# MrGiovanni/R-Super

Hardware: AMD Instinct MI355X
Metric: CT voxels/sec/node (96³ patch, bs=2/GPU) (higher is better)
Workload: dtype bf16; 1 GPU; R-Super 3D UNet(base 32, 26 classes, BasicBlock/IN) full training step (fwd + masked BCE + Dice loss + bwd + clip + AdamW + EMA), 96^3 patches, batch 2/GPU (BASELINE.json configs[1]); global_batch=2, patch=96, parallelism=dp1, sanity_checks_form=device-side flags read one step late (train_ddp.StepGuard)

## Files before the change

include/rsuper_hip.h:

```cpp
#ifndef RSUPER_HIP_H
#define RSUPER_HIP_H
#include <stddef.h>
#include <stdint.h>
#ifdef __cplusplus
extern "C" {
#endif

#define RSUPER_F32 0
#define RSUPER_BF16 1
#define RSUPER_OK 0
#define RSUPER_ERR_ARG 1
#define RSUPER_ERR_LAUNCH 2
#define RSUPER_ERR_UNSUPPORTED 3
#define RSUPER_ERR_NO_DEVICE 4

const char* rsuper_version(void);
int rsuper_device_check(void);


size_t rsuper_conv3_packed_elems(int dtype, int ka, int kb, int n_cols, int bn);

int rsuper_conv3_pack_weights(int dtype, int mode, const float* wa, const float* wb, int ka, int kb, int na, int nb,
                              int bn, void* packed, void* stream);

// ... 177 lines not shown
int rsuper_mask_op(uint8_t* a, const uint8_t* b, long V, int op , void* stream);

int rsuper_unpack_bits(const uint8_t* packed, uint8_t* out, int B, int P, int C, long V, void* stream);
int rsuper_timer_event_create(void** ev);
int rsuper_timer_event_record(void* ev, void* stream);
int rsuper_timer_event_elapsed_ms(void* a, void* b, float* ms);
int rsuper_timer_event_destroy(void* ev);

int rsuper_unpack_bits_sel(const uint8_t* packed, uint8_t* out, int B, int P, int C, long V, const uint8_t* flags, const uint8_t* force, void* stream);
int rsuper_plane_any_bits(const uint8_t* packed, int B, int P, int C, long V, uint8_t* flags, void* stream);
int rsuper_zero_where(float* x, const uint8_t* m, long V, void* stream);
int rsuper_count(const uint8_t* m, long V, unsigned int* count, void* stream);

long rsuper_detection_workspace_bytes(int planes);
int rsuper_detection(const float* x, int planes, int Di, int Hi, int Wi, int Do, int Ho, int Wo, const double* thresholds, int nthr, int erode,
                     long long* volumes, double* max_prob, void* workspace, void* stream);
int rsuper_organ_mask_u8(const uint8_t* pred, int C, int D, int H, int W, int n, const int* lesion, const int* organ_a, const int* organ_b,
                         uint8_t* out, void* stream);
int rsuper_organ_mask_f32(const float* pred, int C, int D, int H, int W, int n, const int* lesion, const int* organ_a, const int* organ_b,
                          float* out, void* stream);
long rsuper_largest_component_workspace_bytes(int D, int H, int W);
int rsuper_largest_component(const void* mask, int is_u8, int D, int H, int W, uint8_t* out, void* workspace, void* stream);

int rsuper_surface_codes(const uint8_t* gt, const uint8_t* pred, int planes, int D, int H, int W, uint8_t* codes_gt, uint8_t* codes_pred,
                         int* bbox, long long* counts, void* stream);
long rsuper_edt3_workspace_bytes(int nz, int ny, int nx);
int rsuper_edt3(const uint8_t* codes, int Dc, int Hc, int Wc, int z0, int y0, int x0, int nz, int ny, int nx, double s0, double s1, double s2,
                double* out, void* workspace, long workspace_bytes, void* stream);
int rsuper_surfel_gather(const uint8_t* codes, int Dc, int Hc, int Wc, int z0, int y0, int x0, int nz, int ny, int nx, const double* sqdist,
                         const double* table, double* dist, double* area, long long* count, long capacity, void* stream);

#define RSUPER_AFFINE_MAX_VOLUMES 3
#define RSUPER_AFFINE_MAX_PLANES 64
int rsuper_affine_crop(const float* theta, const float* img, float* img_out, int B, int Ci, int D, int H, int W, int nvol,
                       const uint8_t* const* vols, uint8_t* const* vols_out, const int* planes, int d, int h, int w, const int* offsets,
                       void* stream);

#define RSUPER_BLUR_MAX_RADIUS 5
long rsuper_intensity_augment_workspace_bytes(int B, int D, int H, int W);
int rsuper_intensity_augment_launches(int B, const int* flags);
int rsuper_intensity_augment(const float* img, float* out, int B, int D, int H, int W, const int* flags, const float* scalars, const int* radius,
                             const float* taps, const unsigned long long* seeds, const float* noise, void* workspace, long workspace_bytes,
                             void* stream);

int rsuper_grad_sqnorm(int n, void* const* host_g, const size_t* host_numel, double* total_sq, void* stream);
int rsuper_clip_scale(int n, void* const* host_g, const size_t* host_numel, float max_norm, const double* total_sq, void* stream);
int rsuper_adamw_ema_step(int n, void* const* host_p, void* const* host_g, void* const* host_m, void* const* host_v,
                          void* const* host_ema, const size_t* host_numel, float lr, float beta1, float beta2, float eps,
                          float weight_decay, int step, float ema_alpha, float max_norm, const double* total_sq, void* stream);
int rsuper_adamw_ema_step_dyn(int n, void* const* host_p, void* const* host_g, void* const* host_m, void* const* host_v,
                              void* const* host_ema, const size_t* host_numel, float beta1, float beta2, float eps, float weight_decay,
                              float max_norm, const double* total_sq, const float* dyn, void* stream);

#ifdef __cplusplus
}
#endif
#endif
```

r-super_amd/csrc/api.hip:

```cpp
#include <string.h>
#include <math.h>
#include <stdlib.h>
#include "common.hpp"
#include "kernels.hpp"
#include "misc.hpp"
#include "loss.hpp"
#include "morph.hpp"
#include "optim.hpp"
#include "../../include/rsuper_hip.h"

#define ST(s) ((hipStream_t)(s))

static inline bool dt_ok(int dt) { return dt == RS_F32 || dt == RS_BF16; }
static inline bool ch_ok(int C, int ld) { return C >= 0 && (C % 8) == 0 && (ld % 8) == 0 && ld >= C; }
static inline bool bn_ok(int bn) { return bn == 32 || bn == 64 || bn == 96 || bn == 128; }
static inline int ntiles_for(int n_cols, int bn) { const int per = bn / 32; return ((n_cols + bn - 1) / bn) * per; }
static inline int pack_cols(int mode, int na, int nb) { return mode == 1 ? (nb ? (nb & 0xFFFF) : na) : na + nb; }
static inline bool pack_range_ok(int mode, int na, int nb) { return mode != 1 || nb == 0 || ((nb >> 16) % 32 == 0 && (nb & 0xFFFF) > 0 && (nb >> 16) + (nb & 0xFFFF) <= na); }

#include "igemm_plan.hpp"

template <typename F>
static int for_chunks(int n, void* const* p, void* const* g, void* const* m, void* const* v, void* const* e, const size_t* numel, F f) {
    for (int i0 = 0; i0 < n; i0 += RS_MT_MAX) {
// ... 713 lines not shown
int rsuper_plane_any(const uint8_t* m, long planes, long V, uint8_t* flags, void* stream) {
    if (!m || !flags || planes <= 0 || V <= 0 || ((uintptr_t)m & 15) || (V & 15 && planes > 1)) return RS_ERR_ARG;
    return rs_launch_plane_any(m, planes, V, flags, ST(stream));
}
int rsuper_mask_op(uint8_t* a, const uint8_t* b, long V, int op, void* stream) {
    if (!a || !b || op < 0 || op > 2) return RS_ERR_ARG;
    return rs_launch_mask_op(a, b, V, op, ST(stream));
}
int rsuper_zero_where(float* x, const uint8_t* m, long V, void* stream) {
    if (!x || !m) return RS_ERR_ARG;
    return rs_launch_zero_where(x, m, V, ST(stream));
}
int rsuper_count(const uint8_t* m, long V, unsigned int* count, void* stream) {
    if (!m || !count) return RS_ERR_ARG;
    return rs_launch_count(m, V, count, ST(stream));
}

int rsuper_grad_sqnorm(int n, void* const* host_g, const size_t* host_numel, double* total_sq, void* stream) {
    if (n <= 0 || !host_g || !host_numel || !total_sq) return RS_ERR_ARG;
    int first = 1;
    const int rc = for_chunks(n, nullptr, host_g, nullptr, nullptr, nullptr, host_numel, [&](const MTChunk& c) {
        const int r = rs_launch_sqnorm(c, total_sq, first, ST(stream));
        first = 0;
        return r;
    });
    if (rc == RS_OK && first) return rs_launch_zero_bytes(total_sq, sizeof(double), ST(stream));
    return rc;
}
int rsuper_clip_scale(int n, void* const* host_g, const size_t* host_numel, float max_norm, const double* total_sq, void* stream) {
    if (n <= 0 || !host_g || !host_numel || !total_sq) return RS_ERR_ARG;
    return for_chunks(n, nullptr, host_g, nullptr, nullptr, nullptr, host_numel, [&](const MTChunk& c) { return rs_launch_scale(c, max_norm, total_sq, ST(stream)); });
}
int rsuper_adamw_ema_step(int n, void* const* host_p, void* const* host_g, void* const* host_m, void* const* host_v,
                          void* const* host_ema, const size_t* host_numel, float lr, float beta1, float beta2, float eps,
                          float weight_decay, int step, float ema_alpha, float max_norm, const double* total_sq, void* stream) {
    if (n <= 0 || !host_p || !host_g || !host_m || !host_v || !host_numel || step < 1) return RS_ERR_ARG;
    AdamParams a;
    a.lr = lr; a.beta1 = beta1; a.beta2 = beta2; a.eps = eps; a.wd = weight_decay;
    a.step_size = (float)((double)lr / (1.0 - pow((double)beta1, (double)step)));
    a.sqrt_bc2 = (float)sqrt(1.0 - pow((double)beta2, (double)step));
    a.ema_alpha = ema_alpha; a.max_norm = max_norm; a.dyn = nullptr;
    return for_chunks(n, host_p, host_g, host_m, host_v, host_ema, host_numel, [&](const MTChunk& c) { return rs_launch_adamw_ema(c, a, total_sq, ST(stream)); });
}
int rsuper_adamw_ema_step_dyn(int n, void* const* host_p, void* const* host_g, void* const* host_m, void* const* host_v,
                              void* const* host_ema, const size_t* host_numel, float beta1, float beta2, float eps, float weight_decay,
                              float max_norm, const double* total_sq, const float* dyn, void* stream) {
    if (n <= 0 || !host_p || !host_g || !host_m || !host_v || !host_numel || !dyn) return RS_ERR_ARG;
    AdamParams a;
    a.lr = 0.f; a.beta1 = beta1; a.beta2 = beta2; a.eps = eps; a.wd = weight_decay;
    a.step_size = 0.f; a.sqrt_bc2 = 1.f; a.ema_alpha = 0.f; a.max_norm = max_norm; a.dyn = dyn;
    return for_chunks(n, host_p, host_g, host_m, host_v, host_ema, host_numel, [&](const MTChunk& c) { return rs_launch_adamw_ema(c, a, total_sq, ST(stream)); });
}

}
```

r-super_amd/csrc/optim.hip:

```cpp
#include "common.hpp"
#include "optim.hpp"

namespace {

__device__ __forceinline__ int find_tensor(const MTChunk& c, int blk, int& local) {
    int lo = 0, hi = c.n;
    while (hi - lo > 1) { const int mid = (lo + hi) >> 1; if (c.blk_start[mid] <= blk) lo = mid; else hi = mid; }
    local = blk - c.blk_start[lo];
    return lo;
}

constexpr int MT_ELEMS = 256 * 4 * 4;

__global__ __launch_bounds__(256) void sqnorm_kernel(MTChunk c, double* partial) {
    int local; const int ti = find_tensor(c, blockIdx.x, local);
    const float* g = (const float*)c.g[ti];
    const size_t n = c.numel[ti], base = (size_t)local * MT_ELEMS;
    float s = 0.f;
    if (base + MT_ELEMS <= n && (((uintptr_t)(g + base)) & 15) == 0) {
        const float4* g4 = (const float4*)(g + base);
#pragma unroll
        for (int k = 0; k < MT_ELEMS / 1024; ++k) { const float4 v = g4[threadIdx.x + 256 * k]; s += v.x * v.x + v.y * v.y + v.z * v.z + v.w * v.w; }
    } else {
#pragma unroll
        for (int k = 0; k < MT_ELEMS / 1024; ++k) {
            const size_t i = base + (size_t)(threadIdx.x + 256 * k) * 4;
            const float x = i < n ? g[i] : 0.f, y = i + 1 < n ? g[i + 1] : 0.f, z = i + 2 < n ? g[i + 2] : 0.f, w = i + 3 < n ? g[i + 3] : 0.f;
            s += x * x + y * y + z * z + w * w;
        }
    }
    s = wave_sum(s);
    __shared__ float red[4];
    if ((threadIdx.x & 63) == 0) red[threadIdx.x >> 6] = s;
    __syncthreads();
    if (threadIdx.x == 0) partial[blockIdx.x] = (double)red[0] + (double)red[1] + (double)red[2] + (double)red[3];
}

__global__ __launch_bounds__(256) void sqnorm_reduce_kernel(const double* partial, int n, double* total, int first) {
    __shared__ double red[256];
    double s = 0.0;
    for (int i = threadIdx.x; i < n; i += 256) s += partial[i];
    red[threadIdx.x] = s;
    __syncthreads();
    for (int o = 128; o > 0; o >>= 1) {
        if ((int)threadIdx.x < o) red[threadIdx.x] += red[threadIdx.x + o];
        __syncthreads();
    }
    if (threadIdx.x == 0) *total = first ? red[0] : *total + red[0];
}

__global__ __launch_bounds__(256) void adamw_ema_kernel(MTChunk c, AdamParams a, const double* total_sq) {
    int local; const int ti = find_tensor(c, blockIdx.x, local);
    float* p = (float*)c.p[ti]; const float* g = (const float*)c.g[ti];
    float* m = (float*)c.m[ti]; float* v = (float*)c.v[ti]; float* e = (float*)c.ema[ti];
    const size_t n = c.numel[ti], base = (size_t)local * MT_ELEMS;
    if (a.dyn) { a.lr = a.dyn[0]; a.step_size = a.dyn[1]; a.sqrt_bc2 = a.dyn[2]; a.ema_alpha = a.dyn[3]; }
    float coef = 1.f;
    if (total_sq) {
        const float norm = (float)sqrt(*total_sq);
        if (!(norm <= 3.0e38f)) return;
        coef = fminf(a.max_norm / (norm + 1e-6f), 1.f);
    }
    for (size_t i = base + threadIdx.x; i < base + MT_ELEMS && i < n; i += 256) {
        const float gi = g[i] * coef;
        float pi = p[i] * (1.f - a.lr * a.wd);
        const float mi = a.beta1 * m[i] + (1.f - a.beta1) * gi;
        const float vi = a.beta2 * v[i] + (1.f - a.beta2) * gi * gi;
        const float denom = sqrtf(vi) / a.sqrt_bc2 + a.eps;
        pi -= a.step_size * (mi / denom);
        p[i] = pi; m[i] = mi; v[i] = vi;
        if (e) e[i] = a.ema_alpha * e[i] + (1.f - a.ema_alpha) * pi;
    }
}

__global__ __launch_bounds__(256) void scale_kernel(MTChunk c, float max_norm, const double* total_sq) {
    int local; const int ti = find_tensor(c, blockIdx.x, local);
    float* g = (float*)c.g[ti];
    const size_t n = c.numel[ti], base = (size_t)local * MT_ELEMS;
    const float coef = fminf(max_norm / ((float)sqrt(*total_sq) + 1e-6f), 1.f);
    for (size_t i = base + threadIdx.x; i < base + MT_ELEMS && i < n; i += 256) g[i] *= coef;
}

__global__ __launch_bounds__(256) void zero_bytes_kernel(unsigned char* p, size_t bytes) {
    const size_t nv = bytes / 16, stride = (size_t)gridDim.x * 256;
    for (size_t i = (size_t)blockIdx.x * 256 + threadIdx.x; i < nv; i += stride) ((uint4*)p)[i] = make_uint4(0, 0, 0, 0);
    if (blockIdx.x == 0) for (size_t i = nv * 16 + threadIdx.x; i < bytes; i += 256) p[i] = 0;
}

}

int rs_launch_zero_bytes(void* p, size_t bytes, hipStream_t st) {
    if (!bytes) return RS_OK;
    const size_t nv = bytes / 16;
    size_t blocks = (nv + 255) / 256;
    if (blocks < 1) blocks = 1;
    if (blocks > 4096) blocks = 4096;
    const bool aligned = (((uintptr_t)p) & 15) == 0;
    if (!aligned) return RS_ERR_ARG;
    hipLaunchKernelGGL(zero_bytes_kernel, dim3((unsigned)blocks), dim3(256), 0, st, (unsigned char*)p, bytes);
    return rs_check_launch();
}
int rs_mt_blocks(size_t numel) { return (int)((numel + MT_ELEMS - 1) / MT_ELEMS); }

int rs_launch_sqnorm(const MTChunk& c, double* total, int first, hipStream_t st) {
    static double* ws[16] = {};
    constexpr int WS_BLOCKS = 1 << 16;
    int dev = 0;
    if (hipGetDevice(&dev) != hipSuccess || dev < 0 || dev >= 16) return RS_ERR_LAUNCH;
    if (!ws[dev] && hipMalloc((void**)&ws[dev], (size_t)WS_BLOCKS * sizeof(double)) != hipSuccess) return RS_ERR_LAUNCH;
    const int blocks = c.blk_start[c.n];
    if (blocks > WS_BLOCKS) return RS_ERR_UNSUPPORTED;
    hipLaunchKernelGGL(sqnorm_kernel, dim3(blocks), dim3(256), 0, st, c, ws[dev]);
    hipLaunchKernelGGL(sqnorm_reduce_kernel, dim3(1), dim3(256), 0, st, (const double*)ws[dev], blocks, total, first);
    return rs_check_launch();
}
int rs_launch_adamw_ema(const MTChunk& c, const AdamParams& a, const double* total_sq, hipStream_t st) {
    hipLaunchKernelGGL(adamw_ema_kernel, dim3(c.blk_start[c.n]), dim3(256), 0, st, c, a, total_sq);
    return rs_check_launch();
}
int rs_launch_scale(const MTChunk& c, float max_norm, const double* total_sq, hipStream_t st) {
    hipLaunchKernelGGL(scale_kernel, dim3(c.blk_start[c.n]), dim3(256), 0, st, c, max_norm, total_sq);
    return rs_check_launch();
}
```

r-super_amd/csrc/optim.hpp:

```cpp
#pragma once
#include <hip/hip_runtime.h>
#include <stddef.h>
#include <stdint.h>

#define RS_MT_MAX 36
struct MTChunk {
    int n;
    void* p[RS_MT_MAX]; void* g[RS_MT_MAX]; void* m[RS_MT_MAX]; void* v[RS_MT_MAX]; void* ema[RS_MT_MAX];
    size_t numel[RS_MT_MAX];
    int blk_start[RS_MT_MAX + 1];
};
struct AdamParams {
    float lr, beta1, beta2, eps, wd;
    float step_size;
    float sqrt_bc2;
    float ema_alpha;
    float max_norm;
    const float* dyn;
};
int rs_mt_blocks(size_t numel);
int rs_launch_sqnorm(const MTChunk& c, double* total, int first, hipStream_t st);
int rs_launch_zero_bytes(void* p, size_t bytes, hipStream_t st);
int rs_launch_adamw_ema(const MTChunk& c, const AdamParams& a, const double* total_sq, hipStream_t st);
int rs_launch_scale(const MTChunk& c, float max_norm, const double* total_sq, hipStream_t st);
```

r-super_amd/hip/lib.py:

```python
import ctypes
import os
from ctypes import c_int, c_long, c_longlong, c_size_t, c_float, c_double, c_void_p, c_uint32, c_uint

_HERE = os.path.dirname(os.path.abspath(__file__))
SO_PATH = os.path.join(os.path.dirname(_HERE), 'csrc', 'librsuper_hip.so')

F32, BF16 = 0, 1
BLUR_MAX_RADIUS = 5
_LIB = None

P = c_void_p
_SIGS = {
    'rsuper_version': (ctypes.c_char_p, []),
    'rsuper_device_check': (c_int, []),
    'rsuper_conv3_packed_elems': (c_size_t, [c_int] * 5),
    'rsuper_conv3_pack_weights': (c_int, [c_int, c_int, P, P, c_int, c_int, c_int, c_int, c_int, P, P]),
    'rsuper_conv3_pack_weights_batch': (c_int, [c_int, c_int, P, P, P, P, P, P]),
    'rsuper_conv3_tiles': (c_int, [c_int] * 3),
    'rsuper_conv3_variant': (c_int, [c_int]),
    'rsuper_conv3_wgrad2_min_tiles': (c_int, [c_int]),
    'rsuper_conv3_plan': (c_int, [c_int] * 11 + [P]),
    'rsuper_conv3_box_bn': (c_int, [c_int] * 6),
    'rsuper_conv3_kd_bn': (c_int, [c_int] * 8),
    'rsuper_conv3_set_workspace': (c_int, [P, c_size_t]),
# ... 61 lines not shown
    'rsuper_depthwise3_rows': (c_int, [c_long]),
    'rsuper_depthwise3_fwd': (c_int, [P, P, P, c_int, c_int, c_int, c_int, c_int, c_int, P]),
    'rsuper_depthwise3_wgrad': (c_int, [P, P, P, P, c_int, c_int, c_int, c_int, c_int, P]),
    'rsuper_seg_from_sums': (c_int, [P, P, c_int, c_int, c_size_t, c_double, P, P, P]),
    'rsuper_report_from_sums': (c_int, [P, P, c_int, c_int, c_int, c_size_t, c_int, P, P, c_double, c_double, c_int, P, c_int, c_int, P, P, P]),
    'rsuper_plane_partials_bwd': (c_int, [P, c_size_t, P, P, P, P, P, P, c_int, c_int, c_size_t, P]),
    'rsuper_sigmoid_mask': (c_int, [P, P, P, c_size_t, P]),
    'rsuper_window_accumulate': (c_int, [P, P] + [c_int] * 11 + [P]),
    'rsuper_window_normalize': (c_int, [P, P, P, P, c_long, c_int, c_int, c_int, P]),
    'rsuper_dilate_volume': (c_int, [P, P, P, c_long, c_int, c_int, c_int, c_int, P]),
    'rsuper_dilate_volume_sparse': (c_int, [P, P, P, P, c_long, c_int, c_int, c_int, c_int, P]),
    'rsuper_ball_workspace_floats': (c_long, [c_int, c_int, c_int, c_int]),
    'rsuper_ball_conv_argmax': (c_int, [P, c_int, c_int, c_int, c_int, c_float, P, P, P, P]),
    'rsuper_insert_ball': (c_int, [P, c_int, c_int, c_int, c_int, c_int, c_int, c_int, c_int, P, P]),
    'rsuper_insert_ball_at': (c_int, [P, c_int, c_int, c_int, P, c_int, c_int, P, P]),
    'rsuper_radix_hist': (c_int, [P, P, c_long, c_uint32, c_int, P, P]),
    'rsuper_topk_mark': (c_int, [P, P, c_long, c_uint32, c_uint, P, P]),
    'rsuper_compact': (c_int, [P, P, c_long, P, P, P, P]),
    'rsuper_rank_weights': (c_int, [P, P, c_uint, c_float, c_float, P, P]),
    'rsuper_rank_assign': (c_int, [P, c_uint, c_float, c_float, P, P]),
    'rsuper_topk_select': (c_int, [P, P, c_long, c_uint, P, P, P]),
    'rsuper_topk_select_multi': (c_int, [P, P, c_long, P, c_int, P, P, c_int, P]),
    'rsuper_plane_any': (c_int, [P, c_long, c_long, P, P]),
    'rsuper_guard_range': (c_int, [P, c_size_t, c_float, c_float, P, P]),
    'rsuper_guard_consistency': (c_int, [P, P, P, c_int, c_int, P, P]),
    'rsuper_mask_op': (c_int, [P, P, c_long, c_int, P]),
    'rsuper_unpack_bits': (c_int, [P, P, c_int, c_int, c_int, c_long, P]),
    'rsuper_timer_event_create': (c_int, [P]),
    'rsuper_timer_event_record': (c_int, [P, P]),
    'rsuper_timer_event_elapsed_ms': (c_int, [P, P, P]),
    'rsuper_timer_event_destroy': (c_int, [P]),
    'rsuper_unpack_bits_sel': (c_int, [P, P, c_int, c_int, c_int, c_long, P, P, P]),
    'rsuper_plane_any_bits': (c_int, [P, c_int, c_int, c_int, c_long, P, P]),
    'rsuper_zero_where': (c_int, [P, P, c_long, P]),
    'rsuper_count': (c_int, [P, c_long, P, P]),
    'rsuper_detection_workspace_bytes': (c_long, [c_int]),
    'rsuper_detection': (c_int, [P, c_int, c_int, c_int, c_int, c_int, c_int, c_int, P, c_int, c_int, P, P, P, P]),
    'rsuper_organ_mask_u8': (c_int, [P, c_int, c_int, c_int, c_int, c_int, P, P, P, P, P]),
    'rsuper_organ_mask_f32': (c_int, [P, c_int, c_int, c_int, c_int, c_int, P, P, P, P, P]),
    'rsuper_largest_component_workspace_bytes': (c_long, [c_int, c_int, c_int]),
    'rsuper_largest_component': (c_int, [P, c_int, c_int, c_int, c_int, P, P, P]),
    'rsuper_affine_crop': (c_int, [P, P, P, c_int, c_int, c_int, c_int, c_int, c_int, P, P, P, c_int, c_int, c_int, P, P]),
    'rsuper_intensity_augment_workspace_bytes': (c_long, [c_int] * 4),
    'rsuper_intensity_augment_launches': (c_int, [c_int, P]),
    'rsuper_intensity_augment': (c_int, [P, P, c_int, c_int, c_int, c_int, P, P, P, P, P, P, P, c_long, P]),
    'rsuper_surface_codes': (c_int, [P, P, c_int, c_int, c_int, c_int, P, P, P, P, P]),
    'rsuper_edt3_workspace_bytes': (c_long, [c_int, c_int, c_int]),
    'rsuper_edt3': (c_int, [P] + [c_int] * 9 + [c_double] * 3 + [P, P, c_long, P]),
    'rsuper_surfel_gather': (c_int, [P] + [c_int] * 9 + [P, P, P, P, P, c_long, P]),
    'rsuper_grad_sqnorm': (c_int, [c_int, P, P, P, P]),
    'rsuper_clip_scale': (c_int, [c_int, P, P, c_float, P, P]),
    'rsuper_adamw_ema_step': (c_int, [c_int, P, P, P, P, P, P, c_float, c_float, c_float, c_float, c_float, c_int, c_float, c_float, P, P]),
    'rsuper_adamw_ema_step_dyn': (c_int, [c_int, P, P, P, P, P, P, c_float, c_float, c_float, c_float, c_float, P, P, P]),
}

IGEMM_CLASSIC, IGEMM_PC, IGEMM_WS, IGEMM_KD, IGEMM_BOX = range(5)

ERR = {1: 'RSUPER_ERR_ARG', 2: 'RSUPER_ERR_LAUNCH', 3: 'RSUPER_ERR_UNSUPPORTED', 4: 'RSUPER_ERR_NO_DEVICE'}


class RSuperHipError(RuntimeError):
    pass


def lib():
    global _LIB
    if _LIB is None:
        if not os.path.exists(SO_PATH):
            raise RSuperHipError(f'{SO_PATH} not found: build it with `make -C r-super_amd/csrc` '
                                 f'(or python -c "import __graft_entry__ as g; g.build()"). There is no CPU fallback.')
        L = ctypes.CDLL(SO_PATH)
        for name, (res, args) in _SIGS.items():
            fn = getattr(L, name)
            fn.restype, fn.argtypes = res, args
        if 'RSUPER_IGEMM_VARIANT' in os.environ:
            L.rsuper_conv3_variant(int(os.environ['RSUPER_IGEMM_VARIANT']))
        _LIB = L
    return _LIB


def exported_symbols():
    return sorted(_SIGS)


def check(rc, what):
    if rc != 0:
        raise RSuperHipError(f'{what} failed: {ERR.get(rc, rc)}')


def require_device():
    check(lib().rsuper_device_check(), 'rsuper_device_check (MI355X / gfx950 required)')
```

r-super_amd/hip/ops.py:

```python
import ctypes
import os

import torch
import torch.nn.functional as F

from . import lib as _l

EPS = 1e-4
_DT = {torch.float32: _l.F32, torch.bfloat16: _l.BF16}


def use_tr():
    return int(os.environ.get('RSUPER_WGRAD_TR', '1'))


_DEV_INDEX = None


def _stream():
    global _DEV_INDEX
    if _DEV_INDEX is None:
        _DEV_INDEX = torch.cuda.current_device()
    return torch._C._cuda_getCurrentRawStream(_DEV_INDEX)

# ... 39 lines not shown
def part_buffer(dtype, dims, n_cols, bn, device, fill=None, epi=0, mixed=False):
    shape = (dims[0], igemm_plan(dtype, epi, dims, n_cols, bn, mixed)[4], n_cols, 2)
    if fill is None:
        return torch.empty(shape, device=device, dtype=torch.float32)
    return torch.full(shape, fill, device=device, dtype=torch.float32)


def stats_finalize(part, cnt, mode=0, split=0):
    N, nblk, C, _ = part.shape
    out = torch.empty((N, C, 2), device=part.device, dtype=torch.float32)
    _l.check(_L().rsuper_stats_finalize(_ptr(part), N, nblk, C, float(cnt), EPS, mode, split, _ptr(out), _stream()), 'stats_finalize')
    if split:
        flat = out.view(-1)
        return flat[:N * split * 2].view(N, split, 2), flat[N * split * 2:].view(N, C - split, 2)
    return out


def pack_weights(dtype, mode, wa, wb, ka, kb, na, nb, bn):
    dt = _DT[dtype]
    n = _L().rsuper_conv3_packed_elems(dt, ka, kb, na + nb, bn)
    out = torch.empty((n,), device=wa.device, dtype=dtype)
    _l.check(_L().rsuper_conv3_pack_weights(dt, mode, _ptr(wa), _ptr(wb), ka, kb, na, nb, bn, _ptr(out), _stream()), 'pack_weights')
    return out


def _spec_cols(sp):
    return (sp[6] & 0xFFFF) if (sp[0] == 1 and sp[6]) else sp[5] + sp[6]


def _pack_desc(dtype, specs):
    dt = _DT[dtype]
    n = len(specs)
    offs = [0]
    for sp in specs:
        offs.append(offs[-1] + _L().rsuper_conv3_packed_elems(dt, sp[3], sp[4], _spec_cols(sp), sp[7]))
    desc = (ctypes.c_int * (6 * n))(*[v for sp in specs for v in (sp[0], sp[3], sp[4], sp[5], sp[6], sp[7])])
    wa = (ctypes.c_void_p * n)(*[sp[1].data_ptr() for sp in specs])
    wb = (ctypes.c_void_p * n)(*[(sp[2].data_ptr() if sp[2] is not None else None) for sp in specs])
    oe = (ctypes.c_size_t * n)(*offs[:-1])
    return (dt, n, desc, wa, wb, oe), offs


def _pack_launch(args, offs, dtype, device):
    buf = torch.empty((offs[-1],), device=device, dtype=dtype)
    _l.check(_L().rsuper_conv3_pack_weights_batch(*args, _ptr(buf), _stream()), 'pack_weights_batch')
    return [buf[offs[i]:offs[i + 1]] for i in range(len(offs) - 1)]


def pack_weights_batch(dtype, specs):
    return _pack_launch(*_pack_desc(dtype, specs), dtype, specs[0][1].device)


_BLOCK_PACK_CACHE = {}


def block_packs(w1, w2, ws, Ca, Cb, dtype, tiles_total, with_backward, dims, mixed=False):
    key = (w1.data_ptr(), w2.data_ptr(), 0 if ws is None else ws.data_ptr(), w1.shape[0], Ca, Cb, dtype, tiles_total, with_backward, dims, mixed,
           rs_variant_epoch())
    ent = _BLOCK_PACK_CACHE.get(key)
    if ent is None:
        specs, bns = block_pack_specs(w1, w2, ws, Ca, Cb, dtype, tiles_total, with_backward, dims, mixed)
        if len(_BLOCK_PACK_CACHE) > 1024:
            _BLOCK_PACK_CACHE.clear()
        ent = _BLOCK_PACK_CACHE[key] = _pack_desc(dtype, specs) + (bns,)
    return _pack_launch(ent[0], ent[1], dtype, w1.device), ent[2]


def rs_variant_epoch():
    return (_L().rsuper_conv3_variant(-1), os.environ.get('RSUPER_SPLIT_DGRAD', '1'))


def block_pack_specs(w1, w2, ws, Ca, Cb, dtype, tiles_total, with_backward, dims=None, mixed=False):
    Cout, Cin = w1.shape[0], Ca + Cb
    has_sc = ws is not None
    nc1 = Cout * (2 if has_sc else 1)
    bn1, bn2 = pick_bn(nc1, dtype, tiles_total, dims, epi=0, mixed=mixed), pick_bn(Cout, dtype, tiles_total, dims, epi=0)
    specs = [(0, w1, ws, Ca, Cb, Cout, Cout if has_sc else 0, bn1), (0, w2, None, Cout, 0, Cout, 0, bn2)]
    bns = [bn1, bn2]
    if with_backward:
        bnd2, bnd1 = pick_bn(Cout, dtype, tiles_total, dims, epi=1), pick_bn(Cin, dtype, tiles_total, dims, epi=1)
        specs += [(1, w2, None, Cout, 0, Cout, 0, bnd2)]
        bns += [bnd2]
        if split_dgrad_sources(Ca, Cb, dtype, tiles_total, bnd1):
            bna, bnb = pick_bn(Ca, dtype, tiles_total, dims, epi=1), pick_bn(Cb, dtype, tiles_total, dims, epi=1)
            specs += [(1, w1, ws, Cout, Cout if has_sc else 0, Cin, Ca, bna), (1, w1, ws, Cout, Cout if has_sc else 0, Cin, (Ca << 16) | Cb, bnb)]
            bns += [bna, bnb]
        else:
            specs += [(1, w1, ws, Cout, Cout if has_sc else 0, Cin, 0, bnd1)]
            bns += [bnd1]
    return specs, bns


def split_dgrad_sources(Ca, Cb, dtype, tiles_total, bn_joint):
    if os.environ.get('RSUPER_SPLIT_DGRAD', '1') == '0' or dtype == torch.float32 or not Cb:
        return False
    return bn_joint == 32 and Ca % 32 == 0 and Cb % 64 == 0 and tiles_total is not None and tiles_total >= 2048


class Src:

    def __init__(self, t, C=None, off=0, mr=None):
        self.t, self.off, self.mr = t, off, mr
        self.ld = t.shape[-1]
        self.C = self.ld - off if C is None else C

    def args(self):
        return (_ptr(self.t, self.off), self.ld, self.C, _ptr(self.mr))


_NONE = (None, 0, 0, None)


class KernelTimer:

    def __init__(self, fenced=None):
        self.fenced = (os.environ.get('RSUPER_TIMER_FENCED', '0') == '1') if fenced is None else bool(fenced)
        self.records = []
# ... 1157 lines not shown
```

r-super_amd/training/utils.py:

```python
import ctypes
import math

import torch

from ..hip import lib as _l
from ..hip.ops import _stream


def _ptr_array(tensors):
    return (ctypes.c_void_p * len(tensors))(*[t.data_ptr() for t in tensors])


class FusedAdamWEMA(torch.optim.Optimizer):

    def __init__(self, params, lr=6e-4, betas=(0.9, 0.999), eps=1e-5, weight_decay=0.05):
        super().__init__(params, dict(lr=lr, betas=tuple(betas), eps=eps, weight_decay=weight_decay))
        self._total_sq = None

    def _state_for(self, p):
        st = self.state[p]
        if not st:
            st['step'] = 0
            st['exp_avg'] = torch.zeros_like(p, memory_format=torch.preserve_format)
            st['exp_avg_sq'] = torch.zeros_like(p, memory_format=torch.preserve_format)
        elif not isinstance(st['step'], int):
            st['step'] = int(st['step'].item()) if torch.is_tensor(st['step']) else int(st['step'])
        return st

    def load_state_dict(self, state_dict):
        super().load_state_dict(state_dict)
        for st in self.state.values():
            if 'step' in st and not isinstance(st['step'], int):
                st['step'] = int(st['step'].item()) if torch.is_tensor(st['step']) else int(st['step'])
            for k in ('exp_avg', 'exp_avg_sq'):
                if k in st:
                    st[k] = st[k].float().contiguous()

    @torch.no_grad()
    def grad_sqnorm(self):
        from ..hip import ops as _ops
        _ops.join_side()
        ps = [p for g in self.param_groups for p in g['params'] if p.grad is not None]
        if self._total_sq is None:
            self._total_sq = torch.zeros(1, device=ps[0].device, dtype=torch.float64)
        gs = [p.grad for p in ps]
        numel = (ctypes.c_size_t * len(gs))(*[g.numel() for g in gs])
        _l.check(_l.lib().rsuper_grad_sqnorm(len(gs), _ptr_array(gs), numel, self._total_sq.data_ptr(), _stream()), 'grad_sqnorm')
        return self._total_sq

    @torch.no_grad()
    def fused_step(self, max_norm=None, ema_params=None, ema_alpha=0.0):
        from ..hip import ops as _ops
        _ops.join_side()
        total = self.grad_sqnorm() if max_norm is not None else None
        ema_of = {}
        if ema_params is not None:
            all_p = [p for g in self.param_groups for p in g['params']]
            ema_of = {id(p): e for p, e in zip(all_p, ema_params)}
        for group in self.param_groups:
            ps = [p for p in group['params'] if p.grad is not None]
            if not ps:
                continue
            for p in ps:
                assert p.is_contiguous() and p.grad.is_contiguous() and p.dtype == torch.float32 and p.grad.dtype == torch.float32
            sts = [self._state_for(p) for p in ps]
            steps = {st['step'] for st in sts}
            assert len(steps) == 1, 'parameters of one group must share the step count'
            step = steps.pop() + 1
            for st in sts:
                st['step'] = step
            b1, b2 = group['betas']
            emas = [ema_of[id(p)] for p in ps] if ema_params is not None else None
            numel = (ctypes.c_size_t * len(ps))(*[p.numel() for p in ps])
            dyn = getattr(self, 'dyn', None)
            if dyn is not None:
                assert len(self.param_groups) == 1 and max_norm is not None
                _l.check(_l.lib().rsuper_adamw_ema_step_dyn(
                    len(ps), _ptr_array(ps), _ptr_array([p.grad for p in ps]), _ptr_array([st['exp_avg'] for st in sts]),
                    _ptr_array([st['exp_avg_sq'] for st in sts]), _ptr_array(emas) if emas is not None else None, numel,
                    b1, b2, group['eps'], group['weight_decay'], float(max_norm), total.data_ptr(), dyn.data_ptr(), _stream()), 'adamw_ema_step_dyn')
                continue
            _l.check(_l.lib().rsuper_adamw_ema_step(
                len(ps), _ptr_array(ps), _ptr_array([p.grad for p in ps]), _ptr_array([st['exp_avg'] for st in sts]),
                _ptr_array([st['exp_avg_sq'] for st in sts]), _ptr_array(emas) if emas is not None else None, numel,
                group['lr'], b1, b2, group['eps'], group['weight_decay'], step, float(ema_alpha),
                float(max_norm if max_norm is not None else 0.0), total.data_ptr() if total is not None else None, _stream()),
                'adamw_ema_step')
        _ops.WEIGHTS_EPOCH += 1
        return total.sqrt().float() if total is not None else None

    @torch.no_grad()
    def step(self, closure=None):
        loss = closure() if closure is not None else None
        self.fused_step()
        return loss


def clip_grad_norm_(parameters, max_norm, optimizer=None):
    ps = [p for p in parameters if p.grad is not None]
    gs = [p.grad for p in ps]
    total = torch.zeros(1, device=gs[0].device, dtype=torch.float64)
    numel = (ctypes.c_size_t * len(gs))(*[g.numel() for g in gs])
    arr = _ptr_array(gs)
    _l.check(_l.lib().rsuper_grad_sqnorm(len(gs), arr, numel, total.data_ptr(), _stream()), 'grad_sqnorm')
    _l.check(_l.lib().rsuper_clip_scale(len(gs), arr, numel, float(max_norm), total.data_ptr(), _stream()), 'clip_scale')
    return total.sqrt().float()


def get_optimizer(args, net):
    root = net.module if hasattr(net, 'module') else net
    params = [p for p in root.parameters()]
    name = args.optimizer.lower()
    if name == 'adamw':
        return FusedAdamWEMA(params, lr=args.base_lr, betas=tuple(args.betas), eps=1e-5, weight_decay=args.weight_decay)
    if name == 'sgd':
        return torch.optim.SGD(params, lr=args.base_lr, momentum=args.momentum, weight_decay=args.weight_decay)
    if name == 'adam':
        return torch.optim.Adam(params, lr=args.base_lr, betas=tuple(args.betas), weight_decay=args.weight_decay)
    raise ValueError(f'Unknown optimizer: {args.optimizer}')


def exp_lr_scheduler_with_warmup(optimizer, epoch, warmup_epoch, max_epoch):
    for g in optimizer.param_groups:
        g.setdefault('base_lr', g['lr'])
    if warmup_epoch and 0 <= epoch <= warmup_epoch:
        lr_mult = math.exp(10.0 * (float(epoch) / float(warmup_epoch) - 1.0))
        if epoch == warmup_epoch:
            lr_mult = 1.0
    else:
        lr_mult = (1.0 - epoch / max_epoch) ** 0.9
    for g in optimizer.param_groups:
        g['lr'] = g['base_lr'] * lr_mult
    return optimizer.param_groups[0]['lr']


def ema_alpha_for_step(alpha, global_step):
    return min((1 - 1 / (global_step + 1)), alpha)


@torch.no_grad()
def update_ema_variables(model, ema_model, alpha, global_step):
    from ..hip import ops as _ops
# ... 17 lines not shown
```

Baseline: 172.6 million voxels/s.

## Fuse AdamW/EMA update with bf16 conv weight fragment packing into persistent arenas

Adds an optimizer kernel that, for 3x3x3 conv weights, updates params/moments/EMA per 32x32 channel tile, stages the new weights as bf16 in shared memory, and writes them straight into the packed igemm fragment layouts. Block packs now live in persistent per-block arenas that are only repacked when stale, so the next forward can skip the separate weight-pack kernel launches and the extra weight read. This adds bookkeeping for arena validity (epochs, tensor versions, weakrefs) and a split between packed and plain parameters, with correctness risk if the staleness tracking misses an update.

```diff
diff --git a/include/rsuper_hip.h b/include/rsuper_hip.h
--- a/include/rsuper_hip.h
+++ b/include/rsuper_hip.h
@@ -253,6 +253,14 @@
                               void* const* host_ema, const size_t* host_numel, float beta1, float beta2, float eps, float weight_decay,
                               float max_norm, const double* total_sq, const float* dyn, void* stream);
 
+size_t rsuper_adamw_pack_entry_bytes(void);
+int rsuper_adamw_ema_pack_step(int n, void* const* host_p, void* const* host_g, void* const* host_m, void* const* host_v, void* const* host_ema,
+                               const void* host_table, const void* dev_table, float lr, float beta1, float beta2, float eps, float weight_decay,
+                               int step, float ema_alpha, float max_norm, const double* total_sq, void* stream);
+int rsuper_adamw_ema_pack_step_dyn(int n, void* const* host_p, void* const* host_g, void* const* host_m, void* const* host_v, void* const* host_ema,
+                                   const void* host_table, const void* dev_table, float beta1, float beta2, float eps, float weight_decay,
+                                   float max_norm, const double* total_sq, const float* dyn, void* stream);
+
 #ifdef __cplusplus
 }
 #endif
diff --git a/r-super_amd/csrc/api.hip b/r-super_amd/csrc/api.hip
--- a/r-super_amd/csrc/api.hip
+++ b/r-super_amd/csrc/api.hip
@@ -789,4 +789,63 @@
     return for_chunks(n, host_p, host_g, host_m, host_v, host_ema, host_numel, [&](const MTChunk& c) { return rs_launch_adamw_ema(c, a, total_sq, ST(stream)); });
 }
 
-}
+static int adamw_pack_impl(int n, void* const* host_p, void* const* host_g, void* const* host_m, void* const* host_v, void* const* host_ema,
+                           const void* host_table, const void* dev_table, const AdamParams& a, const double* total_sq, void* stream) {
+    if (n <= 0 || !host_p || !host_g || !host_m || !host_v || !host_table || !dev_table) return RS_ERR_ARG;
+    const PackEntry* ht = (const PackEntry*)host_table;
+    auto al16 = [](const void* q) { return q && (((uintptr_t)q) & 15) == 0; };
+    for (int i = 0; i < n; ++i) {
+        const PackEntry& en = ht[i];
+        if (en.cout <= 0 || en.cin <= 0 || (en.cout % 32) || (en.cin % 32) || en.ndest < 1 || en.ndest > RS_PACK_DEST_MAX) return RS_ERR_UNSUPPORTED;
+        if (!al16(host_p[i]) || !al16(host_g[i]) || !al16(host_m[i]) || !al16(host_v[i]) || (host_ema && !al16(host_ema[i]))) return RS_ERR_UNSUPPORTED;
+        const int ct = en.cout / 32, it = en.cin / 32;
+        for (int d = 0; d < en.ndest; ++d) {
+            const PackDest& ds = en.d[d];
+            if (!al16(ds.out) || (ds.mode != 0 && ds.mode != 1) || ds.ntiles <= 0 || ds.nt_cnt <= 0 || ds.nt_cnt > ds.ntiles || ds.ch_base < 0) return RS_ERR_ARG;
+            const int chunks = (ds.mode == 0 ? it : ct) + ds.ch_base, nt_hi = (ds.mode == 0 ? ct : it) - 1 + ds.nt_base;
+            if (ds.mode == 0 && (ds.nt_base < 0 || nt_hi >= ds.nt_cnt)) return RS_ERR_ARG;
+            if (ds.mode == 1 && ds.nt_base > 0) return RS_ERR_ARG;
+            if ((long long)chunks * 27 * 2 * ds.ntiles * 64 * 8 > ds.elems) return RS_ERR_ARG;
+        }
+    }
+    for (int i0 = 0; i0 < n; i0 += RS_MT_MAX) {
+        MTChunk c;
+        memset(&c, 0, sizeof(c));
+        c.n = n - i0 < RS_MT_MAX ? n - i0 : RS_MT_MAX;
+        int blk = 0;
+        for (int i = 0; i < c.n; ++i) {
+            const PackEntry& en = ht[i0 + i];
+            c.p[i] = host_p[i0 + i]; c.g[i] = host_g[i0 + i]; c.m[i] = host_m[i0 + i]; c.v[i] = host_v[i0 + i]; c.ema[i] = host_ema ? host_ema[i0 + i] : nullptr;
+            c.numel[i] = (size_t)en.cout * en.cin * 27;
+            c.blk_start[i] = blk;
+            blk += (en.cout / 32) * (en.cin / 32);
+        }
+        c.blk_start[c.n] = blk;
+        const int rc = rs_launch_adamw_ema_pack(c, a, total_sq, (const PackEntry*)dev_table + i0, ST(stream));
+        if (rc) return rc;
+    }
+    return RS_OK;
+}
+size_t rsuper_adamw_pack_entry_bytes(void) { return sizeof(PackEntry); }
+int rsuper_adamw_ema_pack_step(int n, void* const* host_p, void* const* host_g, void* const* host_m, void* const* host_v, void* const* host_ema,
+                               const void* host_table, const void* dev_table, float lr, float beta1, float beta2, float eps, float weight_decay,
+                               int step, float ema_alpha, float max_norm, const double* total_sq, void* stream) {
+    if (step < 1) return RS_ERR_ARG;
+    AdamParams a;
+    a.lr = lr; a.beta1 = beta1; a.beta2 = beta2; a.eps = eps; a.wd = weight_decay;
+    a.step_size = (float)((double)lr / (1.0 - pow((double)beta1, (double)step)));
+    a.sqrt_bc2 = (float)sqrt(1.0 - pow((double)beta2, (double)step));
+    a.ema_alpha = ema_alpha; a.max_norm = max_norm; a.dyn = nullptr;
+    return adamw_pack_impl(n, host_p, host_g, host_m, host_v, host_ema, host_table, dev_table, a, total_sq, stream);
+}
+int rsuper_adamw_ema_pack_step_dyn(int n, void* const* host_p, void* const* host_g, void* const* host_m, void* const* host_v, void* const* host_ema,
+                                   const void* host_table, const void* dev_table, float beta1, float beta2, float eps, float weight_decay,
+                                   float max_norm, const double* total_sq, const float* dyn, void* stream) {
+    if (!dyn) return RS_ERR_ARG;
+    AdamParams a;
+    a.lr = 0.f; a.beta1 = beta1; a.beta2 = beta2; a.eps = eps; a.wd = weight_decay;
+    a.step_size = 0.f; a.sqrt_bc2 = 1.f; a.ema_alpha = 0.f; a.max_norm = max_norm; a.dyn = dyn;
+    return adamw_pack_impl(n, host_p, host_g, host_m, host_v, host_ema, host_table, dev_table, a, total_sq, stream);
+}
+
+}
diff --git a/r-super_amd/csrc/optim.hip b/r-super_amd/csrc/optim.hip
--- a/r-super_amd/csrc/optim.hip
+++ b/r-super_amd/csrc/optim.hip
@@ -49,27 +49,106 @@
     if (threadIdx.x == 0) *total = first ? red[0] : *total + red[0];
 }
 
+__device__ __forceinline__ bool adamw_prologue(AdamParams& a, const double* total_sq, float& coef) {
+    if (a.dyn) { a.lr = a.dyn[0]; a.step_size = a.dyn[1]; a.sqrt_bc2 = a.dyn[2]; a.ema_alpha = a.dyn[3]; }
+    coef = 1.f;
+    if (total_sq) {
+        const float norm = (float)sqrt(*total_sq);
+        if (!(norm <= 3.0e38f)) return false;
+        coef = fminf(a.max_norm / (norm + 1e-6f), 1.f);
+    }
+    return true;
+}
+__device__ __forceinline__ void adamw_elem(const AdamParams& a, float coef, float g, float& pi, float& mi, float& vi) {
+#pragma clang fp contract(off)
+    const float gi = g * coef;
+    mi = fmaf(1.f - a.beta1, gi, a.beta1 * mi);
+    vi = fmaf(gi, (1.f - a.beta2) * gi, a.beta2 * vi);
+    const float denom = sqrtf(vi) / a.sqrt_bc2 + a.eps;
+    pi = fmaf(pi, fmaf(-a.lr, a.wd, 1.f), -(a.step_size * (mi / denom)));
+}
+__device__ __forceinline__ float ema_elem(const AdamParams& a, float e, float pi) {
+#pragma clang fp contract(off)
+    return (1.f - a.ema_alpha) * pi + a.ema_alpha * e;
+}
+
 __global__ __launch_bounds__(256) void adamw_ema_kernel(MTChunk c, AdamParams a, const double* total_sq) {
     int local; const int ti = find_tensor(c, blockIdx.x, local);
     float* p = (float*)c.p[ti]; const float* g = (const float*)c.g[ti];
     float* m = (float*)c.m[ti]; float* v = (float*)c.v[ti]; float* e = (float*)c.ema[ti];
     const size_t n = c.numel[ti], base = (size_t)local * MT_ELEMS;
-    if (a.dyn) { a.lr = a.dyn[0]; a.step_size = a.dyn[1]; a.sqrt_bc2 = a.dyn[2]; a.ema_alpha = a.dyn[3]; }
-    float coef = 1.f;
-    if (total_sq) {
-        const float norm = (float)sqrt(*total_sq);
-        if (!(norm <= 3.0e38f)) return;
-        coef = fminf(a.max_norm / (norm + 1e-6f), 1.f);
-    }
+    float coef;
+    if (!adamw_prologue(a, total_sq, coef)) return;
     for (size_t i = base + threadIdx.x; i < base + MT_ELEMS && i < n; i += 256) {
-        const float gi = g[i] * coef;
-        float pi = p[i] * (1.f - a.lr * a.wd);
-        const float mi = a.beta1 * m[i] + (1.f - a.beta1) * gi;
-        const float vi = a.beta2 * v[i] + (1.f - a.beta2) * gi * gi;
-        const float denom = sqrtf(vi) / a.sqrt_bc2 + a.eps;
-        pi -= a.step_size * (mi / denom);
+        float pi = p[i], mi = m[i], vi = v[i];
+        adamw_elem(a, coef, g[i], pi, mi, vi);
         p[i] = pi; m[i] = mi; v[i] = vi;
-        if (e) e[i] = a.ema_alpha * e[i] + (1.f - a.ema_alpha) * pi;
+        if (e) e[i] = ema_elem(a, e[i], pi);
+    }
+}
+
+constexpr int PK_RS = 32 * 27 + 2;
+__global__ __launch_bounds__(256) void adamw_ema_pack_kernel(MTChunk c, AdamParams a, const double* total_sq, const PackEntry* tab) {
+    __shared__ bf16_t sm[32 * PK_RS];
+    int local; const int ti = find_tensor(c, blockIdx.x, local);
+    float* p = (float*)c.p[ti]; const float* g = (const float*)c.g[ti];
+    float* m = (float*)c.m[ti]; float* v = (float*)c.v[ti]; float* e = (float*)c.ema[ti];
+    float coef;
+    if (!adamw_prologue(a, total_sq, coef)) return;
+    const PackEntry* en = tab + ti;
+    const int cin = en->cin, nit = cin >> 5, ct = local / nit, it = local - ct * nit;
+    const size_t row0 = ((size_t)ct * 32 * cin + (size_t)it * 32) * 27, rstride = (size_t)cin * 27;
+    const int tid = threadIdx.x;
+    constexpr int UB = 3;
+#pragma unroll 1
+    for (int k0 = 0; k0 < 27; k0 += UB) {
+        float4 gq[UB], pq[UB], mq[UB], vq[UB], eq[UB];
+        size_t off[UB];
+        int at[UB];
+#pragma unroll
+        for (int u = 0; u < UB; ++u) {
+            const int idx = tid + (k0 + u) * 256, r = idx / 216, o = (idx - r * 216) * 4;
+            off[u] = row0 + (size_t)r * rstride + o;
+            at[u] = r * PK_RS + o;
+            gq[u] = *(const float4*)(g + off[u]); pq[u] = *(const float4*)(p + off[u]);
+            mq[u] = *(const float4*)(m + off[u]); vq[u] = *(const float4*)(v + off[u]);
+            if (e) eq[u] = *(const float4*)(e + off[u]);
+        }
+#pragma unroll
+        for (int u = 0; u < UB; ++u) {
+            adamw_elem(a, coef, gq[u].x, pq[u].x, mq[u].x, vq[u].x);
+            adamw_elem(a, coef, gq[u].y, pq[u].y, mq[u].y, vq[u].y);
+            adamw_elem(a, coef, gq[u].z, pq[u].z, mq[u].z, vq[u].z);
+            adamw_elem(a, coef, gq[u].w, pq[u].w, mq[u].w, vq[u].w);
+            *(float4*)(p + off[u]) = pq[u]; *(float4*)(m + off[u]) = mq[u]; *(float4*)(v + off[u]) = vq[u];
+            if (e) {
+                eq[u].x = ema_elem(a, eq[u].x, pq[u].x); eq[u].y = ema_elem(a, eq[u].y, pq[u].y);
+                eq[u].z = ema_elem(a, eq[u].z, pq[u].z); eq[u].w = ema_elem(a, eq[u].w, pq[u].w);
+                *(float4*)(e + off[u]) = eq[u];
+            }
+            *(uint32_t*)(sm + at[u]) = f2bf2(pq[u].x, pq[u].y);
+            *(uint32_t*)(sm + at[u] + 2) = f2bf2(pq[u].z, pq[u].w);
+        }
+    }
+    __syncthreads();
+    const int lane = tid & 63, nl = lane & 31, kq = (lane >> 5) * 8;
+    for (int d = 0; d < en->ndest; ++d) {
+        const PackDest& ds = en->d[d];
+        const int mode = ds.mode;
+        const int ch = (mode == 0 ? it : ct) + ds.ch_base, nt = (mode == 0 ? ct : it) + ds.nt_base;
+        if (nt < 0 || nt >= ds.nt_cnt) continue;
+        bf16_t* dst = (bf16_t*)ds.out;
+        const int ntiles = ds.ntiles;
+        for (int i = tid >> 6; i < 54; i += 4) {
+            const int tap = i >> 1, ks = i & 1, k = ks * 16 + kq;
+            const bf16_t* src = mode == 0 ? sm + nl * PK_RS + k * 27 + tap : sm + k * PK_RS + nl * 27 + (26 - tap);
+            const int js = mode == 0 ? 27 : PK_RS;
+            uint32_t w[4];
+#pragma unroll
+            for (int j = 0; j < 4; ++j) w[j] = (uint32_t)src[(2 * j) * js] | ((uint32_t)src[(2 * j + 1) * js] << 16);
+            const size_t idx = ((((size_t)ch * 27 + tap) * 2 + ks) * ntiles + nt) * 64 + lane;
+            *(uint4*)(dst + idx * 8) = make_uint4(w[0], w[1], w[2], w[3]);
+        }
     }
 }
 
@@ -118,6 +197,10 @@
     hipLaunchKernelGGL(adamw_ema_kernel, dim3(c.blk_start[c.n]), dim3(256), 0, st, c, a, total_sq);
     return rs_check_launch();
 }
+int rs_launch_adamw_ema_pack(const MTChunk& c, const AdamParams& a, const double* total_sq, const PackEntry* tab, hipStream_t st) {
+    hipLaunchKernelGGL(adamw_ema_pack_kernel, dim3(c.blk_start[c.n]), dim3(256), 0, st, c, a, total_sq, tab);
+    return rs_check_launch();
+}
 int rs_launch_scale(const MTChunk& c, float max_norm, const double* total_sq, hipStream_t st) {
     hipLaunchKernelGGL(scale_kernel, dim3(c.blk_start[c.n]), dim3(256), 0, st, c, max_norm, total_sq);
     return rs_check_launch();
diff --git a/r-super_amd/csrc/optim.hpp b/r-super_amd/csrc/optim.hpp
--- a/r-super_amd/csrc/optim.hpp
+++ b/r-super_amd/csrc/optim.hpp
@@ -18,8 +18,19 @@
     float max_norm;
     const float* dyn;
 };
+#define RS_PACK_DEST_MAX 4
+struct PackDest {
+    void* out;
+    long long elems;
+    int mode, ch_base, nt_base, nt_cnt, ntiles, pad;
+};
+struct PackEntry {
+    int cout, cin, ndest, pad;
+    PackDest d[RS_PACK_DEST_MAX];
+};
 int rs_mt_blocks(size_t numel);
 int rs_launch_sqnorm(const MTChunk& c, double* total, int first, hipStream_t st);
 int rs_launch_zero_bytes(void* p, size_t bytes, hipStream_t st);
 int rs_launch_adamw_ema(const MTChunk& c, const AdamParams& a, const double* total_sq, hipStream_t st);
+int rs_launch_adamw_ema_pack(const MTChunk& c, const AdamParams& a, const double* total_sq, const PackEntry* tab, hipStream_t st);
 int rs_launch_scale(const MTChunk& c, float max_norm, const double* total_sq, hipStream_t st);
diff --git a/r-super_amd/hip/lib.py b/r-super_amd/hip/lib.py
--- a/r-super_amd/hip/lib.py
+++ b/r-super_amd/hip/lib.py
@@ -137,7 +137,22 @@
     'rsuper_clip_scale': (c_int, [c_int, P, P, c_float, P, P]),
     'rsuper_adamw_ema_step': (c_int, [c_int, P, P, P, P, P, P, c_float, c_float, c_float, c_float, c_float, c_int, c_float, c_float, P, P]),
     'rsuper_adamw_ema_step_dyn': (c_int, [c_int, P, P, P, P, P, P, c_float, c_float, c_float, c_float, c_float, P, P, P]),
+    'rsuper_adamw_pack_entry_bytes': (c_size_t, []),
+    'rsuper_adamw_ema_pack_step': (c_int, [c_int, P, P, P, P, P, P, P, c_float, c_float, c_float, c_float, c_float, c_int, c_float, c_float, P, P]),
+    'rsuper_adamw_ema_pack_step_dyn': (c_int, [c_int, P, P, P, P, P, P, P, c_float, c_float, c_float, c_float, c_float, P, P, P]),
 }
+
+PACK_DEST_MAX = 4
+
+
+class PackDest(ctypes.Structure):
+    _fields_ = [('out', c_void_p), ('elems', c_longlong), ('mode', c_int), ('ch_base', c_int), ('nt_base', c_int), ('nt_cnt', c_int), ('ntiles', c_int),
+                ('pad', c_int)]
+
+
+class PackEntry(ctypes.Structure):
+    _fields_ = [('cout', c_int), ('cin', c_int), ('ndest', c_int), ('pad', c_int), ('d', PackDest * PACK_DEST_MAX)]
+
 
 IGEMM_CLASSIC, IGEMM_PC, IGEMM_WS, IGEMM_KD, IGEMM_BOX = range(5)
 
diff --git a/r-super_amd/hip/ops.py b/r-super_amd/hip/ops.py
--- a/r-super_amd/hip/ops.py
+++ b/r-super_amd/hip/ops.py
@@ -115,9 +115,67 @@
 
 
 _BLOCK_PACK_CACHE = {}
+FUSED_PACK = os.environ.get('RSUPER_FUSED_PACK', '1') == '1'
+ARENA_GEN = 0
+_ARENA_OF = {}
+
+
+class FragmentArena:
+
+    def __init__(self, specs, offs, dtype, weights):
+        import weakref
+        self.buf = torch.empty((offs[-1],), device=weights[0].device, dtype=dtype)
+        self.views = [self.buf[offs[i]:offs[i + 1]] for i in range(len(offs) - 1)]
+        self.refs = [None if w is None else weakref.ref(w) for w in weights]
+        self.stamp, self.versions = None, None
+        self.entries = {}
+        for sp, view in zip(specs, self.views):
+            mode, wa, wb, ka, kb, na, nb, bn = sp
+            cols = _spec_cols(sp)
+            ntiles = ((cols + bn - 1) // bn) * (bn // 32)
+            noff = (nb >> 16) if mode == 1 else 0
+            for w, ch_base, nt_base in ((wa, 0, -(noff // 32)), (wb, ka // 32 if mode == 1 else 0, na // 32 if mode == 0 else -(noff // 32))):
+                if w is None:
+                    continue
+                en = self.entries.get(w.data_ptr())
+                if en is None:
+                    en = self.entries[w.data_ptr()] = _l.PackEntry(cout=w.shape[0], cin=w.shape[1], ndest=0)
+                en.d[en.ndest] = _l.PackDest(out=view.data_ptr(), elems=view.numel(), mode=mode, ch_base=ch_base, nt_base=nt_base,
+                                             nt_cnt=cols // 32 if mode == 1 else ntiles, ntiles=ntiles)
+                en.ndest += 1
+
+    def weights(self):
+        return [None if r is None else r() for r in self.refs]
+
+    def _versions(self):
+        return tuple(None if w is None else w._version for w in self.weights())
+
+    def current(self):
+        return self.stamp == WEIGHTS_EPOCH and self.versions == self._versions()
+
+    def restamp(self):
+        self.stamp, self.versions = WEIGHTS_EPOCH, self._versions()
+
+
+def _arena_ok(specs, dtype, weights):
+    if not FUSED_PACK or dtype != torch.bfloat16:
+        return False
+    for w in weights:
+        if w is not None and not (w.dim() == 5 and tuple(w.shape[2:]) == (3, 3, 3) and w.is_contiguous() and w.dtype == torch.float32
+                                  and w.shape[0] % 32 == 0 and w.shape[1] % 32 == 0 and w.data_ptr() % 16 == 0):
+            return False
+    uses = {}
+    for sp in specs:
+        if any(v % 32 for v in (sp[3], sp[4], sp[5])) or (sp[0] == 0 and sp[6] % 32) or (sp[0] == 1 and sp[6] and ((sp[6] >> 16) % 32 or (sp[6] & 0xFFFF) % 32)):
+            return False
+        for w in (sp[1], sp[2]):
+            if w is not None:
+                uses[w.data_ptr()] = uses.get(w.data_ptr(), 0) + 1
+    return max(uses.values()) <= _l.PACK_DEST_MAX
 
 
 def block_packs(w1, w2, ws, Ca, Cb, dtype, tiles_total, with_backward, dims, mixed=False):
+    global ARENA_GEN
     key = (w1.data_ptr(), w2.data_ptr(), 0 if ws is None else ws.data_ptr(), w1.shape[0], Ca, Cb, dtype, tiles_total, with_backward, dims, mixed,
            rs_variant_epoch())
     ent = _BLOCK_PACK_CACHE.get(key)
@@ -125,7 +183,23 @@
         specs, bns = block_pack_specs(w1, w2, ws, Ca, Cb, dtype, tiles_total, with_backward, dims, mixed)
         if len(_BLOCK_PACK_CACHE) > 1024:
             _BLOCK_PACK_CACHE.clear()
-        ent = _BLOCK_PACK_CACHE[key] = _pack_desc(dtype, specs) + (bns,)
+            _ARENA_OF.clear()
+            ARENA_GEN += 1
+        args, offs = _pack_desc(dtype, specs)
+        arena = None
+        if with_backward and _arena_ok(specs, dtype, (w1, w2, ws)):
+            arena = FragmentArena(specs, offs, dtype, (w1, w2, ws))
+            ARENA_GEN += 1
+            for w in (w1, w2, ws):
+                if w is not None:
+                    _ARENA_OF[w.data_ptr()] = arena
+        ent = _BLOCK_PACK_CACHE[key] = (args, offs, bns, arena)
+    arena = ent[3]
+    if arena is not None and not torch.cuda.is_current_stream_capturing() and all(a is b for a, b in zip(arena.weights(), (w1, w2, ws))):
+        if not arena.current():
+            _l.check(_L().rsuper_conv3_pack_weights_batch(*ent[0], _ptr(arena.buf), _stream()), 'pack_weights_batch')
+            arena.restamp()
+        return arena.views, ent[2]
     return _pack_launch(ent[0], ent[1], dtype, w1.device), ent[2]
 
 
diff --git a/r-super_amd/training/utils.py b/r-super_amd/training/utils.py
--- a/r-super_amd/training/utils.py
+++ b/r-super_amd/training/utils.py
@@ -29,6 +29,7 @@
 
     def load_state_dict(self, state_dict):
         super().load_state_dict(state_dict)
+        self._split_cache = None
         for st in self.state.values():
             if 'step' in st and not isinstance(st['step'], int):
                 st['step'] = int(st['step'].item()) if torch.is_tensor(st['step']) else int(st['step'])
@@ -57,6 +58,7 @@
         if ema_params is not None:
             all_p = [p for g in self.param_groups for p in g['params']]
             ema_of = {id(p): e for p, e in zip(all_p, ema_params)}
+        stamped = []
         for group in self.param_groups:
             ps = [p for p in group['params'] if p.grad is not None]
             if not ps:
@@ -71,23 +73,64 @@
                 st['step'] = step
             b1, b2 = group['betas']
             emas = [ema_of[id(p)] for p in ps] if ema_params is not None else None
-            numel = (ctypes.c_size_t * len(ps))(*[p.numel() for p in ps])
             dyn = getattr(self, 'dyn', None)
             if dyn is not None:
                 assert len(self.param_groups) == 1 and max_norm is not None
-                _l.check(_l.lib().rsuper_adamw_ema_step_dyn(
-                    len(ps), _ptr_array(ps), _ptr_array([p.grad for p in ps]), _ptr_array([st['exp_avg'] for st in sts]),
-                    _ptr_array([st['exp_avg_sq'] for st in sts]), _ptr_array(emas) if emas is not None else None, numel,
-                    b1, b2, group['eps'], group['weight_decay'], float(max_norm), total.data_ptr(), dyn.data_ptr(), _stream()), 'adamw_ema_step_dyn')
-                continue
-            _l.check(_l.lib().rsuper_adamw_ema_step(
-                len(ps), _ptr_array(ps), _ptr_array([p.grad for p in ps]), _ptr_array([st['exp_avg'] for st in sts]),
-                _ptr_array([st['exp_avg_sq'] for st in sts]), _ptr_array(emas) if emas is not None else None, numel,
-                group['lr'], b1, b2, group['eps'], group['weight_decay'], step, float(ema_alpha),
-                float(max_norm if max_norm is not None else 0.0), total.data_ptr() if total is not None else None, _stream()),
-                'adamw_ema_step')
+            packed = self._arena_split(ps, sts, emas)
+            for sel, tab in ((packed[0], packed[2]), (packed[1], None)):
+                if not sel:
+                    continue
+                qs = [ps[i] for i in sel]
+                args = [len(qs), _ptr_array(qs), _ptr_array([p.grad for p in qs]), _ptr_array([sts[i]['exp_avg'] for i in sel]),
+                        _ptr_array([sts[i]['exp_avg_sq'] for i in sel]), _ptr_array([emas[i] for i in sel]) if emas is not None else None]
+                args += [tab[0], tab[1].data_ptr()] if tab is not None else [(ctypes.c_size_t * len(qs))(*[p.numel() for p in qs])]
+                name = 'rsuper_adamw_ema_pack_step' if tab is not None else 'rsuper_adamw_ema_step'
+                if dyn is not None:
+                    args += [b1, b2, group['eps'], group['weight_decay'], float(max_norm), total.data_ptr(), dyn.data_ptr(), _stream()]
+                    name += '_dyn'
+                else:
+                    args += [group['lr'], b1, b2, group['eps'], group['weight_decay'], step, float(ema_alpha),
+                             float(max_norm if max_norm is not None else 0.0), total.data_ptr() if total is not None else None, _stream()]
+                _l.check(getattr(_l.lib(), name)(*args), name[7:])
+            stamped += packed[3]
         _ops.WEIGHTS_EPOCH += 1
+        for arena in stamped:
+            arena.restamp()
         return total.sqrt().float() if total is not None else None
+
+    def _arena_split(self, ps, sts, emas):
+        from ..hip import ops as _ops
+        everything = ([], list(range(len(ps))), None, [])
+        if not _ops.FUSED_PACK or not _ops._ARENA_OF or (ps[0].is_cuda and torch.cuda.is_current_stream_capturing()):
+            return everything
+        sig = (_ops.ARENA_GEN, tuple(p.grad.data_ptr() for p in ps), None if emas is None else tuple(e.data_ptr() for e in emas))
+        hit = getattr(self, '_split_cache', None)
+        if hit is not None and hit[0] == sig and all(a.current() for a in hit[2]):
+            return hit[1]
+        sel, rest, arenas = [], [], {}
+        for i, p in enumerate(ps):
+            ar = _ops._ARENA_OF.get(p.data_ptr())
+            ts = (p, p.grad, sts[i]['exp_avg'], sts[i]['exp_avg_sq']) + ((emas[i],) if emas is not None else ())
+            if ar is not None and any(w is p for w in ar.weights()) and all(t.data_ptr() % 16 == 0 and t.is_contiguous() for t in ts):
+                if id(ar) not in arenas:
+                    arenas[id(ar)] = (ar, ar.current())
+                if arenas[id(ar)][1]:
+                    sel.append(i)
+                    continue
+            rest.append(i)
+        if not sel:
+            return everything
+        host = (_l.PackEntry * len(sel))(*[_ops._ARENA_OF[ps[i].data_ptr()].entries[ps[i].data_ptr()] for i in sel])
+        assert ctypes.sizeof(_l.PackEntry) == _l.lib().rsuper_adamw_pack_entry_bytes()
+        hit = getattr(self, '_pack_table', None)
+        if hit is None or bytes(hit[0]) != bytes(host):
+            hit = self._pack_table = (host, torch.frombuffer(bytearray(host), dtype=torch.uint8).to(ps[0].device))
+        chosen = {id(ps[i]) for i in sel}
+        involved = [a for a, ok in arenas.values() if ok]
+        done = [a for a in involved if all(w is None or id(w) in chosen for w in a.weights())]
+        out = (sel, rest, hit, done)
+        self._split_cache = (sig, out, involved) if len(done) == len(involved) else None
+        return out
 
     @torch.no_grad()
     def step(self, closure=None):
```

Result: no change. 174.1 million voxels/s, median of 6 (+0.9%).
